# zju3dv/clean-pvnet

Measured on AMD Instinct MI355X. Metric: images/sec RANSAC-vote (480x640, K=9, 512 hyp), higher is better.
Workload: dtype f32; 1 GPU; BASELINE config 3 (cfg3): 480x640, K=9, 512 hypotheses, ~2% foreground, int64 mask, contiguous [B,H,W,K,2] f32 vertex; global batch 64 in contiguous shards of 64 images per GPU; ransac_voting_layer_v3 (+ one RCCL all_gather of [B,K,2] per step for N>1, see extra.exchange); steps cycle over 3 distinct device-resident batches; batch_per_gpu=64, global_batch=64, H=480, W=640, K=9, hn=512, parallelism=batch-sharded x1 (strong scaling: 64 images in total)

## Files before the change

clean-pvnet_amd/csrc/compaction.hpp:

```cpp
#pragma once

struct MaskArgs {
    const void *mask;
    const float *selection;
    int64_t sb, sh, sw;
    int es;
    int contig;
    int mode;
    int W, HW, T;
    int min_num, max_num, cap;
    uint64_t seed;
    int b0;
    int *tn_user;
    int *status;
    int fuse_sub;
    int want_draws;
    const float *seg;
    long long *mask_out;
    int64_t gb, gc, gh, gw;
    int C;
};

constexpr uint32_t kTileNzMask = 0xfffu;

// ... 65 lines not shown

__device__ __forceinline__ float selection_draw(const MaskArgs &a, int b, int p)
{
    if (a.selection) return a.selection[(int64_t)b * a.HW + p];
    return (float)(rng_u32(a.seed, 0u, (uint32_t)(a.b0 + b), (uint32_t)p) >> 8) * 0x1p-24f;
}

__device__ __forceinline__ float list_draw(const MaskArgs &a, int b, int i, int e, const unsigned short *__restrict__ lists ,
                                           const float *__restrict__ draws )
{
    if (draws) return draws[(size_t)i * kTile + e];
    return selection_draw(a, b, i * kTile + (int)lists[(size_t)i * kTile + e]);
}

__device__ __forceinline__ void scan_segments(int *seg)
{
    __syncthreads();
    if (threadIdx.x < 64) {
        const int lane = threadIdx.x;
        const int c = lane < kTileSteps * 4 ? seg[lane] : 0;
        const int inc = wave_incl_scan(c);
        if (lane < kTileSteps * 4) seg[lane] = inc - c;
        if (lane == kTileSteps * 4 - 1) seg[kTileSteps * 4] = inc;
    }
    __syncthreads();
}

template <int ES> struct RawElem;
template <> struct RawElem<1> { typedef uint8_t type; };
template <> struct RawElem<2> { typedef uint16_t type; };
template <> struct RawElem<4> { typedef uint32_t type; };
template <> struct RawElem<8> { typedef uint64_t type; };

template <int ES, bool AHEAD, int MODE , int ST = kElemF32 >
__global__ __launch_bounds__(kBlock) void k_tile_scan(MaskArgs a, uint32_t *__restrict__ tiles,
                                                      unsigned short *__restrict__ tile_list,
                                                      float *__restrict__ tile_draw, int total_tiles)
{
    typedef typename RawElem<ES>::type raw_t;
    __shared__ int seg2[2][kTileSteps * 4 + 1];
    __shared__ int red2[2][4];
    const int lane = lane_id(), wave = threadIdx.x >> 6;
    raw_t cur[AHEAD ? kTileSteps : 1] = {};
    int g = blockIdx.x;
    int b = g / a.T, t = g - b * a.T;
    const int step_b = (int)gridDim.x / a.T, step_t = (int)gridDim.x - step_b * a.T;
    [[maybe_unused]] auto load_tile = [&](raw_t (&dst)[AHEAD ? kTileSteps : 1], int bi, int ti) {
        const raw_t *src = (const raw_t *)a.mask + (int64_t)bi * a.sb + (int64_t)ti * kTile + threadIdx.x;
        if ((ti + 1) * kTile <= a.HW) {
#pragma unroll
            for (int s = 0; s < kTileSteps; ++s) dst[AHEAD ? s : 0] = src[s * kBlock];
        } else {
#pragma unroll
            for (int s = 0; s < kTileSteps; ++s)
                dst[AHEAD ? s : 0] = ti * kTile + s * kBlock + (int)threadIdx.x < a.HW ? src[s * kBlock] : (raw_t)0;
        }
    };
    if constexpr (AHEAD) if (g < total_tiles) load_tile(cur, b, t);
    for (int it = 0; g < total_tiles; ++it) {
        int *seg = seg2[it & 1], *red = red2[it & 1];
        raw_t nxt[AHEAD ? kTileSteps : 1] = {};
        const int gn = g + gridDim.x;
        int bn = b + step_b, tn = t + step_t;
        if (tn >= a.T) { tn -= a.T; ++bn; }
        if constexpr (AHEAD) if (gn < total_tiles) load_tile(nxt, bn, tn);
        unsigned long long m[kTileSteps];
        int pc[kTileSteps];
        int sum = 0;
#pragma unroll
        for (int s = 0; s < kTileSteps; ++s) {
// ... 5 lines not shown
            } else if (p < a.HW) {
                w = mask_weight<ES, ST>(a, b, p);
            }
            m[s] = __ballot(w != 0);
            pc[s] = __popcll(m[s]);
            sum += w;
        }
        if (MODE == 0) sum = wave_total(sum);
        else sum = pc[0] + pc[1] + pc[2] + pc[3] + pc[4] + pc[5] + pc[6] + pc[7];
        if (lane == 0) {
#pragma unroll
            for (int s = 0; s < kTileSteps; ++s) seg[s * 4 + wave] = pc[s];
            red[wave] = sum;
        }
        scan_segments(seg);
        if (threadIdx.x == 0)
            tiles[b * a.T + t] = (uint32_t)seg[kTileSteps * 4] | ((uint32_t)(red[0] + red[1] + red[2] + red[3]) << 12);
        unsigned short *list = tile_list + ((size_t)b * a.T + t) * kTile;
        float *draw = tile_draw + ((size_t)b * a.T + t) * kTile;
        if (seg[kTileSteps * 4] != 0) {
#pragma unroll
            for (int s = 0; s < kTileSteps; ++s)
                if ((m[s] >> lane) & 1ull) {
                    const int r = seg[s * 4 + wave] + __popcll(m[s] & ((1ull << lane) - 1ull));
                    list[r] = (unsigned short)(s * kBlock + threadIdx.x);
                    if (a.want_draws) draw[r] = selection_draw(a, b, t * kTile + s * kBlock + threadIdx.x);
                }
        }
        if constexpr (AHEAD) {
#pragma unroll
            for (int s = 0; s < kTileSteps; ++s) cur[s] = nxt[s];
        }
        g = gn; b = bn; t = tn;
    }
}

typedef float f32x4 __attribute__((ext_vector_type(4)));
typedef long long i64x2 __attribute__((ext_vector_type(2)));
typedef uint32_t u32x2 __attribute__((ext_vector_type(2)));

template <int ST>
__device__ __forceinline__ f32x4 widen_logits4(u32x2 w)
{
    const float2 lo = widen_pair<ST>(w.x), hi = widen_pair<ST>(w.y);
    return f32x4{lo.x, lo.y, hi.x, hi.y};
}

template <bool WRITE_MASK, int ST = kElemF32>
__global__ __launch_bounds__(kBlock) void k_tile_scan_seg2(MaskArgs a, uint32_t *__restrict__ tiles,
                                                           unsigned short *__restrict__ tile_list,
                                                           float *__restrict__ tile_draw)
{
    typedef typename Elem<ST>::raw raw_t;
    __shared__ int seg[8];
    const int g = blockIdx.x;
    const int b = g / a.T, t = g - b * a.T;
    const int lane = lane_id(), wave = threadIdx.x >> 6;
    const raw_t *p0 = (const raw_t *)a.seg + (int64_t)b * a.gb + (int64_t)t * kTile + 4 * threadIdx.x;
    const raw_t *p1 = p0 + a.gc;
    constexpr int kHalf = kTile / 2;
    f32x4 v0[2], v1[2];
    if constexpr (ST == kElemF32) {
#pragma unroll
        for (int s = 0; s < 2; ++s) {
            const bool in = t * kTile + s * kHalf + 4 * (int)threadIdx.x < a.HW;
            v0[s] = in ? __builtin_nontemporal_load((const f32x4 *)(p0 + s * kHalf)) : f32x4{0.f, 0.f, 0.f, 0.f};
// ... 159 lines not shown

__global__ __launch_bounds__(kBlock) void k_tile_subsample(MaskArgs a, uint32_t *__restrict__ tiles,
                                                           unsigned short *__restrict__ tile_list,
                                                           const float *__restrict__ tile_draw)
{
    __shared__ long long redl[4];
    __shared__ int red[8];
    __shared__ int seg[kTileSteps * 4 + 1];
    __shared__ unsigned short keep[kTile];
    const int t = blockIdx.x, b = blockIdx.y;
    const uint32_t w = tiles[b * a.T + t];
    const int nz = (int)(w & kTileNzMask);
    if (nz == 0) return;
    const ImageTotals tot = image_totals(tiles, b, a.T, t, redl, red);
    if (tot.fg <= (long long)a.max_num) return;
    const float prob = (float)a.max_num / (float)tot.fg;
    unsigned short *list = tile_list + ((size_t)b * a.T + t) * kTile;
    const int n = filter_tile_list(a, b, t, nz, prob, tile_list + (size_t)b * a.T * kTile, tile_draw + (size_t)b * a.T * kTile, keep, seg);
    __syncthreads();
    for (int i = threadIdx.x; i < n; i += kBlock) list[i] = keep[i];
    if (threadIdx.x == 0) tiles[b * a.T + t] = (uint32_t)n | (w & ~kTileNzMask);
}

struct VertexArgs {
    const float *vertex;
    int64_t sb, sh, sw, sk, sc;
    int K;
    int vec2;
};

template <int VT> struct VertexRaw { typedef uint2 type; };
template <> struct VertexRaw<kElemF32> { typedef float2 type; };

template <int VT>
__device__ __forceinline__ typename VertexRaw<VT>::type load_vertex(const VertexArgs &v, int b, int y, int x, int vi)
{
    if constexpr (VT == kElemF32) {
        const float *src = v.vertex + (int64_t)b * v.sb + (int64_t)y * v.sh + (int64_t)x * v.sw + (int64_t)vi * v.sk;
        if (v.vec2) return *(const float2 *)src;
        return make_float2(src[0], src[v.sc]);
    } else {
        const uint16_t *src = (const uint16_t *)v.vertex + (int64_t)b * v.sb + (int64_t)y * v.sh + (int64_t)x * v.sw + (int64_t)vi * v.sk;
        if (v.vec2) return make_uint2(*(const uint32_t *)src, 0u);
        return make_uint2(src[0], src[v.sc]);
    }
}

template <int VT>
__device__ __forceinline__ float2 widen_vertex(const VertexArgs &v, typename VertexRaw<VT>::type r)
{
    if constexpr (VT == kElemF32) {
        return r;
    } else {
        typedef typename Elem<VT>::raw raw_t;
        if (v.vec2) return widen_pair<VT>(r.x);
        return make_float2(widen(__builtin_bit_cast(raw_t, (uint16_t)r.x)), widen(__builtin_bit_cast(raw_t, (uint16_t)r.y)));
    }
}

struct HypArgs {
    const int32_t *idxs;
    const int32_t *idxs2;
    int hn, hn_first;
    uint32_t stream, stream2;
    float2 *hyps;
    int *counts;
    int32_t *draws_out;
    int blocks;
    int *surv;
    int *lead;
    int *miss;
};

constexpr int kHypRejectTries = 1 << 12;
constexpr float kSurvMinProb = 1.f / 64.f;
constexpr int kSurvCap = 8192;

__device__ __forceinline__ int select_pixel(const int *prefix, int T, const unsigned short *__restrict__ lists , int t,
                                            size_t *entry = nullptr )
{
    int lo = 0, hi = T - 1;
    while (lo < hi) {
        const int mid = (lo + hi) >> 1;
        if (prefix[mid] > t) hi = mid; else lo = mid + 1;
    }
    const int r = t - (lo ? prefix[lo - 1] : 0);
    const size_t e = (size_t)lo * kTile + r;
    if (entry) *entry = e;
    return lo * kTile + (int)lists[e];
}
// ... 43 lines not shown
        if (fg < (long long)a.min_num) tn = 0;
        const bool sub = a.fuse_sub && fg > (long long)a.max_num;
        const float prob = sub ? (float)a.max_num / (float)fg : 2.f;
        int nsurv = -1;
        if (sub && prob < kSurvMinProb) {
            int *sv = h.surv + (size_t)b * kSurvCap;
            nsurv = 0;
            for (int i = 0; i < a.T; ++i) {
                const int ni = s_prefix[i] - (i ? s_prefix[i - 1] : 0);
                for (int e0 = 0; e0 < ni; e0 += kBlock) {
                    const int e = e0 + threadIdx.x;
                    const bool keep = e < ni && list_draw(a, b, i, e, img_lists, img_draws) < prob;
                    const unsigned long long m = __ballot(keep);
                    __syncthreads();
                    if (lane == 0) red[wave] = __popcll(m);
                    __syncthreads();
                    int off = nsurv;
                    for (int w2 = 0; w2 < wave; ++w2) off += red[w2];
                    off += __popcll(m & ((1ull << lane) - 1ull));
                    if (keep && off < kSurvCap) sv[off] = i * kTile + (int)img_lists[(size_t)i * kTile + e];
                    nsurv += red[0] + red[1] + red[2] + red[3];
                }
            }
            __threadfence_block();
            __syncthreads();
            if (nsurv > kSurvCap) nsurv = -1;
            else if (nsurv < tn) tn = nsurv;
        }

        const int gid = j * kBlock + threadIdx.x;
        if (gid >= v.K * h.hn) return;
        const int vi = gid / h.hn, hi = gid - vi * h.hn;
        const size_t o = ((size_t)b * v.K + vi) * h.hn + hi;
        h.counts[o] = 0;
        if (h.miss) h.miss[o] = 0;
        if (h.lead && hi == 0) {
            int *lw = h.lead + ((size_t)b * v.K + vi) * 8 + 4;
            lw[0] = 0; lw[1] = 0; lw[2] = 0; lw[3] = 0;
        }
        if (tn <= 0) {
            h.hyps[o] = make_float2(0.f, 0.f);
            if (h.draws_out) { h.draws_out[2 * o] = -1; h.draws_out[2 * o + 1] = -1; }
            return;
        }
        const bool first = hi < h.hn_first;
        const int32_t *src = first ? h.idxs : h.idxs2;
        int p0, p1;
        if (src) {
            const int32_t *ip = first ? h.idxs + (((size_t)b * h.hn_first + hi) * v.K + vi) * 2
                                      : h.idxs2 + (((size_t)b * (h.hn - h.hn_first) + (hi - h.hn_first)) * v.K + vi) * 2;
            int t0 = ip[0], t1 = ip[1];
            t0 = t0 < 0 ? 0 : (t0 >= tn ? tn - 1 : t0);
            t1 = t1 < 0 ? 0 : (t1 >= tn ? tn - 1 : t1);
            p0 = select_pixel(s_prefix, a.T, img_lists, t0);
            p1 = select_pixel(s_prefix, a.T, img_lists, t1);
        } else {
            const uint32_t stream = first ? h.stream : h.stream2;
            const uint32_t c = (uint32_t)((first ? hi : hi - h.hn_first) * v.K + vi) * 2u;
            const uint32_t img = (uint32_t)(a.b0 + b);
            if (!sub) {
                p0 = select_pixel(s_prefix, a.T, img_lists, (int)(rng_u32(a.seed, stream, img, c) % (uint32_t)tn));
                p1 = select_pixel(s_prefix, a.T, img_lists, (int)(rng_u32(a.seed, stream, img, c + 1u) % (uint32_t)tn));
            } else if (nsurv >= 0) {
                const int *sv = h.surv + (size_t)b * kSurvCap;
                p0 = sv[rng_u32(a.seed, stream, img, c) % (uint32_t)tn];
                p1 = sv[rng_u32(a.seed, stream, img, c + 1u) % (uint32_t)tn];
            } else {
                p0 = p1 = -1;
                for (int tr = 0; tr < kHypRejectTries && (p0 < 0 || p1 < 0); ++tr) {
                    size_t e;
                    const uint32_t stry = stream + 16u + 4u * (uint32_t)tr;
                    if (p0 < 0) {
                        const int p = select_pixel(s_prefix, a.T, img_lists, (int)(rng_u32(a.seed, stry, img, c) % (uint32_t)total), &e);
                        if ((img_draws ? img_draws[e] : selection_draw(a, b, p)) < prob) p0 = p;
                    }
                    if (p1 < 0) {
                        const int p = select_pixel(s_prefix, a.T, img_lists, (int)(rng_u32(a.seed, stry, img, c + 1u) % (uint32_t)total), &e);
                        if ((img_draws ? img_draws[e] : selection_draw(a, b, p)) < prob) p1 = p;
                    }
                }
                if (p0 < 0 || p1 < 0) {
                    h.hyps[o] = make_float2(0.f, 0.f);
                    if (h.draws_out) { h.draws_out[2 * o] = p0; h.draws_out[2 * o + 1] = p1; }
                    return;
                }
            }
        }
        const int y0 = p0 / a.W, x0 = p0 - y0 * a.W, y1 = p1 / a.W, x1 = p1 - y1 * a.W;
        const typename VertexRaw<VT>::type r0 = load_vertex<VT>(v, b, y0, x0, vi), r1 = load_vertex<VT>(v, b, y1, x1, vi);
        const float2 d0 = widen_vertex<VT>(v, r0), d1 = widen_vertex<VT>(v, r1);
        h.hyps[o] = hypothesis_exact(d0.x, d0.y, (float)x0, (float)y0, d1.x, d1.y, (float)x1, (float)y1);
        if (h.draws_out) { h.draws_out[2 * o] = p0; h.draws_out[2 * o + 1] = p1; }
        return;
    }

    const int t = blockIdx.x - h.blocks;
    const int nz = (int)(tiles[b * a.T + t] & kTileNzMask);
    if (t != 0 && !(a.fuse_sub && t == a.T - 1) && nz == 0) return;
    const unsigned short *my_list = img_lists + (size_t)t * kTile;
    unsigned short mine[kTileSteps];
#pragma unroll
    for (int s = 0; s < kTileSteps; ++s) {
        const int e = s * kBlock + threadIdx.x;
        mine[s] = e < nz ? my_list[e] : (unsigned short)0;
    }
    const ImageTotals tot = image_totals(tiles, b, a.T, t, redl, red);
    if (tot.fg < (long long)a.min_num) {
        if (t == 0 && threadIdx.x == 0) {
            tn_out[b] = 0;
            if (a.tn_user) a.tn_user[b] = 0;
            if (a.status) a.status[b] = PVV_STATUS_SKIPPED;
        }
        return;
    }
    int before = tot.before, tile_n = nz;
    const bool sub = a.fuse_sub && tot.fg > (long long)a.max_num;
    if (sub) {
        const float prob = (float)a.max_num / (float)tot.fg;
        int cnt = 0;
        if (img_draws || a.T > kBlock) {
            for (int i = 0; i < t; ++i) {
                const int ni = (int)(tiles[b * a.T + i] & kTileNzMask);
                for (int e = threadIdx.x; e < ni; e += kBlock)
                    cnt += list_draw(a, b, i, e, img_lists, img_draws) < prob ? 1 : 0;
// ... 40 lines not shown
                }
            }
        }
        before = block_sum(cnt, red);
        __syncthreads();
        tile_n = filter_tile_list(a, b, t, nz, prob, img_lists, img_draws, list, seg);
        __syncthreads();
        if (t == a.T - 1 && threadIdx.x == 0) {
            const int all = before + tile_n;
            tn_out[b] = all < a.cap ? all : a.cap;
            if (a.tn_user) a.tn_user[b] = tn_out[b];
            if (a.status) a.status[b] = PVV_STATUS_SUBSAMPLED | (all > a.cap ? PVV_STATUS_TRUNCATED : 0);
        }
    } else {
        if (t == 0 && threadIdx.x == 0) {
            tn_out[b] = tot.total < a.cap ? tot.total : a.cap;
            if (a.tn_user) a.tn_user[b] = tn_out[b];
            if (a.status) a.status[b] = (tot.fg > (long long)a.max_num ? PVV_STATUS_SUBSAMPLED : 0) |
                                        (tot.total > a.cap ? PVV_STATUS_TRUNCATED : 0);
        }
#pragma unroll
        for (int s = 0; s < kTileSteps; ++s) {
            const int e = s * kBlock + threadIdx.x;
            if (e < nz) list[e] = mine[s];
        }
        __syncthreads();
    }
    const int room = a.cap - before;
    const int n = tile_n < room ? tile_n : (room > 0 ? room : 0);
    constexpr int kKeys = 12;
    for (int li = threadIdx.x; li < n; li += kBlock) {
        const int p = t * kTile + list[li];
        const int y = p / a.W, x = p - y * a.W;
        coords[(size_t)b * a.cap + before + li] = make_float2((float)x, (float)y);
        float2 *drow = dirs + (size_t)b * v.K * a.cap + before + li;
        for (int v0 = 0; v0 < v.K; v0 += kKeys) {
            typename VertexRaw<VT>::type d[kKeys];
#pragma unroll
            for (int u = 0; u < kKeys; ++u)
                if (v0 + u < v.K) d[u] = load_vertex<VT>(v, b, y, x, v0 + u);
#pragma unroll
            for (int u = 0; u < kKeys; ++u)
                if (v0 + u < v.K) {
                    if constexpr (VT == kElemF32) drow[(size_t)(v0 + u) * a.cap] = d[u];
                    else drow[(size_t)(v0 + u) * a.cap] = widen_vertex<VT>(v, d[u]);
                }
        }
    }
}
```

clean-pvnet_amd/csrc/count_prune.hpp:

```cpp
#pragma once

struct LeadArgs {
    const int *tn_arr;
    const float2 *coords;
    const float2 *dirs;
    const float2 *hyps;
    const int *counts;
    int *lead;
    const int *any_staged;
    int K, hn, cap;
    int hstride;
    float kappa, beta, eps;
    int nsplit;
};

constexpr int kLead = 2;

template <uint32_t FIRST>
__global__ __launch_bounds__(kBlock) void k_lead(LeadArgs a)
{
    constexpr uint32_t REST = stage_rest_of(FIRST);
    __shared__ int s_cnt[4], s_idx[4], s_sum[4][4];
    const int vi = blockIdx.x / a.nsplit, split = blockIdx.x - vi * a.nsplit, b = blockIdx.y, bk = b * a.K + vi;
    const int lane = lane_id(), wave = threadIdx.x >> 6;
    constexpr int PC = 4 * kBfPixPerWave;
    if (*a.any_staged == 0) return;
    const int tn = a.tn_arr[b];
    const int nch = (tn + PC - 1) / PC;
    if (tn <= 0 || nch < kStageMinChunks) return;
    constexpr int kTrip = 10;
    const int rem_px = stage_pixels<REST>(tn, nch, PC);
    const int per = (rem_px + a.nsplit - 1) / a.nsplit;
    const int r1 = min(rem_px, (split + 1) * per);
    const float2 *crd = a.coords + (size_t)b * a.cap;
    const float2 *dir = a.dirs + (size_t)bk * a.cap;
    float2 cc[kTrip], dd_[kTrip];
    auto load_trip = [&](int r0) {
#pragma unroll
        for (int u = 0; u < kTrip; ++u) {
            const int r = r0 + u * kBlock;
            cc[u] = dd_[u] = make_float2(0.f, 0.f);
            if (r < r1) {
                const int p = stage_chunk_at<REST>(r / PC) * PC + (r & (PC - 1));
                cc[u] = crd[p];
                dd_[u] = dir[p];
            }
        }
    };
    int r0 = split * per + threadIdx.x;
    load_trip(r0);
    const int *cp = a.counts + (size_t)bk * a.hstride;
    int best = -1, besth = 0x7fffffff;
    for (int h = threadIdx.x; h < a.hn; h += kBlock) {
// ... 63 lines not shown
```

clean-pvnet_amd/csrc/pvnet_vote.hip:

```cpp
#include <hip/hip_runtime.h>

#include <algorithm>
#include <cmath>
#include <cstdio>
#include <cstdlib>
#include <cstring>
#include <mutex>
#include <type_traits>

#include "pvnet_vote.h"

#pragma clang fp contract(off)

#define PVV_EXPORT extern "C" __attribute__((visibility("default")))

namespace {

constexpr int kBlock = 256;
constexpr int kTileSteps = 8;
constexpr int kTile = kBlock * kTileSteps;
constexpr int kFuseSubTiles = 160;
constexpr int kMaxTiles = 16000;
constexpr int kPixPerWave = 64;

// ... 55 lines not shown
Layout make_layout(const pvv_problem *p)
{
    Layout L;
    const size_t HW = (size_t)p->H * p->W;
    L.T = (int)((HW + kTile - 1) / kTile);
    size_t off = 0;
    auto take = [&](size_t bytes) { size_t o = off; off = align_up(off + bytes); return o; };
    L.tiles = take(sizeof(uint32_t) * (size_t)p->B * L.T);
    L.tile_list = take(sizeof(unsigned short) * (size_t)p->B * L.T * kTile);
    L.tile_draw = may_store_draws(p, L.T) ? take(sizeof(float) * (size_t)p->B * L.T * kTile) : 0;
    L.tn = take(sizeof(int) * (size_t)p->B);
    L.surv = take(sizeof(int) * (size_t)p->B * kSurvCap);
    L.coords = take(sizeof(float2) * (size_t)p->B * p->cap);
    L.dirs = take(sizeof(float2) * (size_t)p->B * p->K * p->cap);
    L.hyps = take(sizeof(float2) * (size_t)p->B * p->K * p->hn);
    L.counts = take(sizeof(int) * (size_t)p->B * p->K * p->hn);
    L.sums = take(sizeof(double) * (size_t)p->B * p->K * kRefitSplitMax * 5);
    L.ratio = take(sizeof(float) * (size_t)p->B * p->K);
    L.lead = may_stage(p) ? take(sizeof(int) * 2 * lead_set_words(p)) : 0;
    L.miss = may_stage(p) ? take(sizeof(int) * (size_t)p->B * p->K * p->hn) : 0;
    L.total = off;
    return L;
}

int validate(const pvv_problem *p)
{
    if (!p) return fail(PVV_E_ARG, "problem is NULL");
    if (p->B <= 0 || p->H <= 0 || p->W <= 0 || p->K <= 0 || p->hn <= 0)
        return fail(PVV_E_ARG, "B, H, W, K, hn must be positive");
    if (p->B > kMaxBatchLds) return fail(PVV_E_ARG, "B > 1024: split the batch");
    if (((long long)p->H * p->W + kTile - 1) / kTile > kMaxTiles) return fail(PVV_E_ARG, "H*W too large (more than 16000 tiles of 2048 pixels)");
    if ((long long)p->K * p->hn >= (1ll << 23)) return fail(PVV_E_ARG, "K*hn must be < 2^23");
    if (p->count_kernel < PVV_COUNT_AUTO || p->count_kernel > PVV_COUNT_STAGED_ESTIMATE) return fail(PVV_E_ARG, "unknown count_kernel");
    if (p->flags & ~(PVV_FLAG_DEVICE_RNG | PVV_FLAG_VERTEX_F16 | PVV_FLAG_VERTEX_BF16 | PVV_FLAG_SEG_F16 | PVV_FLAG_SEG_BF16))
        return fail(PVV_E_ARG, "unknown bits in flags");
    if ((p->flags & PVV_FLAG_VERTEX_F16) && (p->flags & PVV_FLAG_VERTEX_BF16))
        return fail(PVV_E_ARG, "flags: PVV_FLAG_VERTEX_F16 and PVV_FLAG_VERTEX_BF16 are exclusive");
    if ((p->flags & PVV_FLAG_SEG_F16) && (p->flags & PVV_FLAG_SEG_BF16))
        return fail(PVV_E_ARG, "flags: PVV_FLAG_SEG_F16 and PVV_FLAG_SEG_BF16 are exclusive");
    if (p->mask_elem_size != 1 && p->mask_elem_size != 2 && p->mask_elem_size != 4 &&
        p->mask_elem_size != 8)
        return fail(PVV_E_ARG, "mask_elem_size must be 1, 2, 4 or 8");
    if (p->cap <= 0 || (long long)p->cap > (long long)p->H * p->W)
        return fail(PVV_E_ARG, "cap must be in [1, H*W]");
    if ((long long)p->B * p->K * p->hn >= (1ll << 31) || (long long)p->B * p->K * p->cap >= (1ll << 40))
        return fail(PVV_E_ARG, "problem too large for one call");
    if (p->singular_policy < PVV_SINGULAR_REFERENCE || p->singular_policy > PVV_SINGULAR_IMAGE_ZERO)
        return fail(PVV_E_ARG, "unknown singular_policy");
    return PVV_OK;
}

int num_cus()
{
    static int cus[64] = {0};
    int dev = 0;
    if (hipGetDevice(&dev) != hipSuccess || dev < 0 || dev >= 64) return 256;
    if (!cus[dev]) {
        hipDeviceProp_t prop;
        int n = 0;
        if (hipGetDeviceProperties(&prop, dev) == hipSuccess) n = prop.multiProcessorCount;
        cus[dev] = n > 0 ? n : 256;
    }
    return cus[dev];
}

int launch_count(const CountArgs &a, hipStream_t st)
{
    const int grid = num_cus() * 8;
// ... 132 lines not shown
    static const double xs[6] = {0.0, 0.585, 1.0, 1.585, 2.0, 3.0}, ys[6] = {0.990, 0.966, 0.957, 0.910, 0.765, 0.50};
    const double x = std::log2(std::max(work, 1.0) / 2.26e10);
    double thr;
    if (x <= xs[0]) thr = ys[0] + (ys[1] - ys[0]) / (xs[1] - xs[0]) * (x - xs[0]);
    else if (x >= xs[5]) thr = ys[5];
    else {
        int i = 0;
        while (x > xs[i + 1]) ++i;
        thr = ys[i] + (ys[i + 1] - ys[i]) * (x - xs[i]) / (xs[i + 1] - xs[i]);
    }
    thr -= 0.1 * std::log2(std::max(p->hn, 512) / 512.0);
    return (float)std::min(0.995, std::max(0.5, thr));
}

double stage_work(const pvv_problem *p, hipStream_t st, float *mean = nullptr, float *max_tn = nullptr)
{
    double sum_tn = -1.0;
    float mt = -1.f;
    const float m = stage_hint_mean(p, st, &mt, &sum_tn);
    if (mean) *mean = m;
    if (max_tn) *max_tn = mt;
    if (m < 0.f || sum_tn < 0.0) return stage_proxy_work(p);
    return (double)p->K * p->hn * sum_tn / kStageProxyFg;
}

bool stage_hint_allows(const pvv_problem *p, hipStream_t st)
{
    if (p->count_kernel != PVV_COUNT_AUTO) return true;
    float max_tn = -1.f, m = -1.f;
    const double work = stage_work(p, st, &m, &max_tn);
    if (work < kStageMinWork) return false;
    if (m < 0.f) return true;
    return m >= stage_hint_threshold(p, work) && max_tn > (float)((kStageMinChunks - 1) * 4 * kBfPixPerWave);
}

Bf16Consts bf16_consts(float thresh)
{
    const double T = (double)thresh, s2 = 1.0 - T * T, kappa = T / std::sqrt(s2);
    const double u = 0x1p-24;
    Bf16Consts fc;
    fc.beta = (float)(1.25 * (33.0 * (1.0 + kappa) + 8.0 / s2) * u / T);
    fc.eps_c = (float)(1.25 * (1.0 + kappa) * 35.0 * u);
    fc.eps0 = (float)(1.5e-6 * (1.0 + kappa));
    fc.kappa = (float)kappa;
    fc.beta2 = (float)(1.25 * (8.0 * (1.0 + kappa) + 8.0 / s2) * u / T);
#ifdef PVV_TUNING
    static const char *dbg = getenv("PVV_DEBUG_BAND_SCALE");
    if (dbg && *dbg) {
        const float k = (float)atof(dbg);
        fc.beta *= k; fc.eps_c *= k; fc.eps0 *= k;
    }
#endif
    return fc;
}

int tuning_int(const char *name, int dflt)
{
#ifdef PVV_TUNING
    static const char *names[32];
    static int vals[32], n = 0;
    for (int i = 0; i < n; ++i) if (!strcmp(names[i], name)) return vals[i] == INT32_MIN ? dflt : vals[i];
    const char *e = getenv(name);
    if (n < 32) { names[n] = name; vals[n] = e && *e ? atoi(e) : INT32_MIN; ++n; }
    return e && *e ? atoi(e) : dflt;
#else
    (void)name;
// ... 38 lines not shown
    const pvv_problem *p = a.p;
    const Layout &L = *a.L;
    char *ws = a.ws;
    hipStream_t st = a.st;
    const Bf16Consts fc = a.fc;
    const float2 *coords = (const float2 *)(ws + L.coords), *dirs = (const float2 *)(ws + L.dirs);
    const float2 *hyps = (const float2 *)(ws + L.hyps) + a.col0;
    int *counts = (int *)(ws + L.counts) + a.col0;
    const int *tn = (const int *)(ws + L.tn);
    int *lead = (int *)(ws + L.lead) + (size_t)a.lead_set * lead_set_words(p);
    StageArgs sa;
    sa.lead = nullptr;
    sa.any_staged = lead + (size_t)p->B * p->K * 8;
    sa.miss = (int *)(ws + L.miss) + a.col0;
    sa.sub_tenth = a.sub_tenth;
    sa.hstride = a.hstride;
    sa.mean = (a.sub_tenth && tuning_int("PVV_PROX", 1) != 0) ? (const float2 *)a.mean : nullptr;
#ifdef PVV_STAMPS
    sa.dbg = tuning_ptr("PVV_DBG_PTR_FILTER");
#endif
    hipLaunchKernelGGL((k_count_bf16<kCountFirst, FIRST>), dim3(a.per_cu_first * num_cus()), dim3(kBlock), 0, st, coords, dirs, hyps, counts, tn,
                       p->B, p->K, p->hn, p->cap, p->inlier_thresh, fc, a.target_first, a.dbg, sa);
    if (int e = check_launch("k_count_bf16<first>")) return e;
    if (int e = mark(p, PVV_MARK_STAGE0, st)) return e;
    LeadArgs la;
    la.tn_arr = tn; la.coords = coords; la.dirs = dirs; la.hyps = hyps; la.counts = counts; la.lead = lead;
    la.K = p->K; la.hn = p->hn; la.cap = p->cap;
    la.hstride = a.hstride > 0 ? a.hstride : p->hn;
    la.kappa = fc.kappa; la.beta = 2.f * fc.beta2; la.eps = 2.f * fc.eps0;
    la.any_staged = sa.any_staged;
    la.nsplit = 16;
    while (la.nsplit > 1 && (long long)p->B * p->K * la.nsplit > 8ll * num_cus()) la.nsplit >>= 1;
    la.nsplit = tuning_int("PVV_LEAD_SPLIT", la.nsplit);
    hipLaunchKernelGGL(k_lead<FIRST>, dim3(p->K * la.nsplit, p->B), dim3(kBlock), 0, st, la);
    if (int e = check_launch("k_lead")) return e;
    if (int e = mark(p, PVV_MARK_PRUNE0, st)) return e;
    sa.lead = lead;
    const long long rest = p->count_kernel == PVV_COUNT_AUTO ? stage_hint_rest_chunks(p, st, stage_rest_of(FIRST)) : -1;
    const bool runs = rest < 0 || rest * p->K >= 2ll * a.target_filter || p->hn > 512;
    if (tuning_int("PVV_FILTER_OLD", runs ? 0 : 1) == 0) {
        hipLaunchKernelGGL(k_count_filter_runs<FIRST>, dim3(tuning_int("PVV_GRID_PER_CU_FILTER", 5) * num_cus()), dim3(kBlock), sizeof(int) * (size_t)p->B, st, coords, dirs,
                           hyps, counts, tn, p->B, p->K, p->hn, p->cap, p->inlier_thresh, fc, a.target_filter, tuning_int("PVV_RUN_R", 0), sa);
        return check_launch("k_count_filter_runs");
    }
    hipLaunchKernelGGL((k_count_bf16<kCountFilter, FIRST>), dim3(a.per_cu_filter * num_cus()), dim3(kBlock), 0, st, coords, dirs, hyps, counts, tn,
                       p->B, p->K, p->hn, p->cap, p->inlier_thresh, fc, a.target_filter, a.dbg, sa);
    return check_launch("k_count_bf16<filter>");
}

struct CountCols {
    int col0 = 0;
    int hstride = 0;
    int lead_set = 0;
    const float *mean = nullptr;
};

int launch_count_bf16(const pvv_problem *p, const Layout &L, char *ws, hipStream_t st, int staged ,
                      const CountCols &cc = CountCols())
{
    const int per_cu_t = tuning_int("PVV_GRID_PER_CU", 0);
    const int items_per_cu = tuning_int("PVV_ITEMS_PER_CU", 5);
    bool few = p->B <= 8;
    if (p->count_kernel == PVV_COUNT_AUTO) {
        double sum_tn = -1.0;
        if (stage_hint_mean(p, st, nullptr, &sum_tn) >= 0.f && sum_tn >= 0.0)
            few = sum_tn / (4 * kBfPixPerWave) * p->K * ((p->hn + 511) / 512) <= 2000.0;
    }
// ... 60 lines not shown
    if (!may_stage(p) || L.lead == 0) return 0;
    if (kind == 1 && stage_hint_allows(p, st)) return 1;
    if (kind == 2 && (p->count_kernel == PVV_COUNT_STAGED_ESTIMATE || (p->count_kernel == PVV_COUNT_AUTO && est_stage_auto(p, st)))) return 2;
    return 0;
}

int launch_count_any(const pvv_problem *p, const Layout &L, char *ws, hipStream_t st, int staged, const CountCols &cc = CountCols())
{
    if (p->ev_count_begin && hipEventRecord((hipEvent_t)p->ev_count_begin, st) != hipSuccess)
        return fail(PVV_E_ARG, "ev_count_begin is not a valid hipEvent_t");
    if (!use_bf16_count(p) && (cc.col0 || cc.hstride)) return fail(PVV_E_ARG, "internal: a column range needs the bf16 count kernel");
    const int e = use_bf16_count(p) ? launch_count_bf16(p, L, ws, st, staged, cc) : launch_count(planar_count_args(p, L, ws), st);
    if (e) return e;
    if (p->ev_count_end && hipEventRecord((hipEvent_t)p->ev_count_end, st) != hipSuccess)
        return fail(PVV_E_ARG, "ev_count_end is not a valid hipEvent_t");
    return PVV_OK;
}

template <int ES, int MODE, int ST = kElemF32>
void launch_scan(const MaskArgs &m, const Layout &L, char *ws, int B, hipStream_t st)
{
    const long long total = (long long)L.T * B;
    uint32_t *tiles = (uint32_t *)(ws + L.tiles);
    unsigned short *lists = (unsigned short *)(ws + L.tile_list);
    float *draws = (float *)(ws + L.tile_draw);
    if (!(m.contig && !m.seg)) {
        hipLaunchKernelGGL((k_tile_scan<ES, false, MODE, ST>), dim3((unsigned)total), dim3(kBlock), 0, st, m, tiles, lists, draws, (int)total);
        return;
    }
    const int per_cu_t = tuning_int("PVV_SCAN_PER_CU", 0);
    long long per_block = 1;
    if (per_cu_t > 0) per_block = (total + (long long)per_cu_t * num_cus() - 1) / ((long long)per_cu_t * num_cus());
    const int grid = (int)((total + per_block - 1) / per_block);
    hipLaunchKernelGGL((k_tile_scan<ES, true, MODE>), dim3(grid), dim3(kBlock), 0, st, m, tiles, lists, draws, (int)total);
}

struct Front {
    MaskArgs m;
    VertexArgs v;
    HypArgs h;
    bool can_subsample;
    bool seg2;
    int vt, st;
    long long *mask_deferred;
};

Front make_front(const pvv_problem *p, int mode, const void *d_mask, const float *d_vertex, const int32_t *d_idxs,
                 const float *d_selection, char *ws, const Layout &L, int32_t *d_tn, const float *d_seg,
                 int64_t *d_mask_out, const int32_t *d_idxs2, int hn_first, uint32_t stream_first, uint32_t stream_rest)
{
    Front f;
    MaskArgs &m = f.m;
    m.mask = d_mask;
    m.seg = d_seg;
    m.mask_out = (long long *)d_mask_out;
    m.gb = p->seg_stride[0]; m.gc = p->seg_stride[1]; m.gh = p->seg_stride[2]; m.gw = p->seg_stride[3];
    m.C = p->seg_classes;
    m.selection = d_selection;
    m.sb = p->mask_stride[0]; m.sh = p->mask_stride[1]; m.sw = p->mask_stride[2];
    m.es = p->mask_elem_size;
    m.contig = (m.sw == 1 && m.sh == p->W) ? 1 : 0;
    m.mode = mode;
    m.W = p->W; m.HW = p->H * p->W; m.T = L.T;
    m.min_num = p->min_num; m.max_num = p->max_num; m.cap = p->cap;
    m.seed = p->seed;
    m.b0 = p->first_image;
    m.tn_user = d_tn;
// ... 584 lines not shown
```

include/pvnet_vote.h:

```cpp
#ifndef PVNET_VOTE_H_
#define PVNET_VOTE_H_

#include <stddef.h>
#include <stdint.h>

#ifdef __cplusplus
extern "C" {
#endif

#define PVV_OK 0
#define PVV_E_ARG (-1)
#define PVV_E_WORKSPACE (-2)

#define PVV_ABI_VERSION 8

int pvv_abi_version(void);
const char *pvv_last_error(void);

int pvv_shutdown(void);


int pvv_generate_hypothesis(const float *d_direct, const float *d_coords,
                            const int32_t *d_idxs, float *d_hypo_pts, int tn,
                            int vn, int hn, void *stream);
// ... 21 lines not shown
                      const float *d_hypo_pts, int32_t *d_counts, int tn,
                      int vn, int hn, float inlier_thresh, void *stream);


typedef struct pvv_problem {
    int32_t B, H, W, K;
    int32_t hn;
    int32_t mask_elem_size;
    int32_t min_num;
    int32_t max_num;
    int32_t cap;
    int32_t singular_policy;
    float inlier_thresh;
    int64_t mask_stride[3];
    int64_t vertex_stride[5];
    uint64_t seed;
    int32_t seg_classes;
    int32_t first_image;
    int64_t seg_stride[4];
    int32_t count_kernel;
    int32_t flags;
    int32_t *d_draws_out;
    void *ev_count_begin;
    void *ev_count_end;
    int32_t *d_status;
    void **ev_marks;
} pvv_problem;

#define PVV_FLAG_DEVICE_RNG 1
#define PVV_FLAG_VERTEX_F16 2
#define PVV_FLAG_VERTEX_BF16 4
#define PVV_FLAG_SEG_F16 8
#define PVV_FLAG_SEG_BF16 16

#define PVV_STATUS_SKIPPED 1
#define PVV_STATUS_SUBSAMPLED 2
#define PVV_STATUS_TRUNCATED 4

#define PVV_MARK_BEGIN 0
#define PVV_MARK_SCAN 1
#define PVV_MARK_COMPACT 2
#define PVV_MARK_COUNT 3
#define PVV_MARK_SELECT 4
#define PVV_MARK_END 5
#define PVV_MARK_STAGE0 6
#define PVV_MARK_PRUNE0 7
#define PVV_N_MARKS 8

#define PVV_COUNT_AUTO 0
#define PVV_COUNT_EXACT 1

#define PVV_COUNT_FULL 2
#define PVV_COUNT_STAGED 3
#define PVV_COUNT_STAGED_ESTIMATE 4

#define PVV_SINGULAR_REFERENCE 0
#define PVV_SINGULAR_ZERO 1
#define PVV_SINGULAR_IMAGE_ZERO 2

int32_t pvv_default_cap(int32_t H, int32_t W, int32_t max_num);

size_t pvv_workspace_bytes(const pvv_problem *p);

int pvv_ransac_voting_v3(const pvv_problem *p, const void *d_mask,
                         const float *d_vertex, const int32_t *d_idxs,
                         const float *d_selection, void *d_workspace,
// ... 44 lines not shown
```

Before: 331,800 images/s.

## Add wide 16-byte mask scan, nontemporal compaction stores, adaptive lead count

```diff
diff --git a/clean-pvnet_amd/csrc/compaction.hpp b/clean-pvnet_amd/csrc/compaction.hpp
--- a/clean-pvnet_amd/csrc/compaction.hpp
+++ b/clean-pvnet_amd/csrc/compaction.hpp
@@ -121,10 +121,107 @@
 template <> struct RawElem<4> { typedef uint32_t type; };
 template <> struct RawElem<8> { typedef uint64_t type; };
 
-template <int ES, bool AHEAD, int MODE , int ST = kElemF32 >
-__global__ __launch_bounds__(kBlock) void k_tile_scan(MaskArgs a, uint32_t *__restrict__ tiles,
-                                                      unsigned short *__restrict__ tile_list,
-                                                      float *__restrict__ tile_draw, int total_tiles)
+typedef unsigned long long u64x2 __attribute__((ext_vector_type(2)));
+constexpr int kWideSteps = kTileSteps / 2;
+
+__device__ __forceinline__ unsigned wave_incl_scan(unsigned v)
+{
+    v += (unsigned)PVV_DPP(0, (int)v, 0x111, 0xf, true);
+    v += (unsigned)PVV_DPP(0, (int)v, 0x112, 0xf, true);
+    v += (unsigned)PVV_DPP(0, (int)v, 0x114, 0xf, true);
+    v += (unsigned)PVV_DPP(0, (int)v, 0x118, 0xf, true);
+    v += (unsigned)PVV_DPP(0, (int)v, 0x142, 0xa, false);
+    v += (unsigned)PVV_DPP(0, (int)v, 0x143, 0xc, false);
+    return v;
+}
+
+template <int MODE>
+__device__ __forceinline__ void tile_scan_wide(const MaskArgs &a, uint32_t *__restrict__ tiles, unsigned short *__restrict__ tile_list,
+                                               float *__restrict__ tile_draw, int total_tiles)
+{
+    static_assert(kWideSteps * 8 <= 32 && 2 * 64 < 256, "four byte-wide counts in one word");
+    __shared__ int seg2[2][kTileSteps * 4 + 1];
+    __shared__ int red2[2][4];
+    const int lane = lane_id(), wave = threadIdx.x >> 6;
+    u64x2 cur[kWideSteps] = {};
+    int g = blockIdx.x;
+    int b = g / a.T, t = g - b * a.T;
+    const int step_b = (int)gridDim.x / a.T, step_t = (int)gridDim.x - step_b * a.T;
+    auto load_tile = [&](u64x2 (&dst)[kWideSteps], int bi, int ti) {
+        const uint64_t *base = (const uint64_t *)a.mask + (int64_t)bi * a.sb + (int64_t)ti * kTile;
+        const uint64_t *src = base + 2 * threadIdx.x;
+        if ((ti + 1) * kTile <= a.HW && ((uintptr_t)base & 15) == 0) {
+#pragma unroll
+            for (int s = 0; s < kWideSteps; ++s) dst[s] = *(const u64x2 *)(src + s * 2 * kBlock);
+        } else {
+#pragma unroll
+            for (int s = 0; s < kWideSteps; ++s) {
+                const int p = ti * kTile + s * 2 * kBlock + 2 * (int)threadIdx.x;
+                dst[s].x = p < a.HW ? src[s * 2 * kBlock] : 0ull;
+                dst[s].y = p + 1 < a.HW ? src[s * 2 * kBlock + 1] : 0ull;
+            }
+        }
+    };
+    if (g < total_tiles) load_tile(cur, b, t);
+    for (int it = 0; g < total_tiles; ++it) {
+        int *seg = seg2[it & 1], *red = red2[it & 1];
+        u64x2 nxt[kWideSteps] = {};
+        const int gn = g + gridDim.x;
+        int bn = b + step_b, tn = t + step_t;
+        if (tn >= a.T) { tn -= a.T; ++bn; }
+        if (gn < total_tiles) load_tile(nxt, bn, tn);
+        unsigned fg = 0u;
+        unsigned packed = 0u;
+        int sum = 0;
+#pragma unroll
+        for (int s = 0; s < kWideSteps; ++s)
+#pragma unroll
+            for (int j = 0; j < 2; ++j) {
+                const uint64_t v = cur[s][j];
+                const int w = MODE == 0 ? (int)(v & 0xFF) : (v == 1 ? 1 : 0);
+                const unsigned f = w != 0 ? 1u : 0u;
+                fg |= f << (2 * s + j);
+                packed += f << (8 * s);
+                sum += w;
+            }
+        const unsigned inc = wave_incl_scan(packed);
+        const unsigned excl = inc - packed;
+        const unsigned tot = (unsigned)__builtin_amdgcn_readlane((int)inc, 63);
+        if (MODE == 0) sum = wave_total(sum);
+        else sum = (int)((tot & 0xff) + ((tot >> 8) & 0xff) + ((tot >> 16) & 0xff) + (tot >> 24));
+        if (lane == 0) {
+#pragma unroll
+            for (int s = 0; s < kTileSteps; ++s) seg[s * 4 + wave] = s < kWideSteps ? (int)((tot >> (8 * s)) & 0xff) : 0;
+            red[wave] = sum;
+        }
+        scan_segments(seg);
+        if (threadIdx.x == 0)
+            tiles[b * a.T + t] = (uint32_t)seg[kTileSteps * 4] | ((uint32_t)(red[0] + red[1] + red[2] + red[3]) << 12);
+        unsigned short *list = tile_list + ((size_t)b * a.T + t) * kTile;
+        float *draw = tile_draw + ((size_t)b * a.T + t) * kTile;
+        if (seg[kTileSteps * 4] != 0 && fg != 0u) {
+#pragma unroll
+            for (int s = 0; s < kWideSteps; ++s) {
+                int r = seg[s * 4 + wave] + (int)((excl >> (8 * s)) & 0xff);
+#pragma unroll
+                for (int j = 0; j < 2; ++j)
+                    if ((fg >> (2 * s + j)) & 1u) {
+                        const int off = s * 2 * kBlock + 2 * (int)threadIdx.x + j;
+                        list[r] = (unsigned short)off;
+                        if (a.want_draws) draw[r] = selection_draw(a, b, t * kTile + off);
+                        ++r;
+                    }
+            }
+        }
+#pragma unroll
+        for (int s = 0; s < kWideSteps; ++s) cur[s] = nxt[s];
+        g = gn; b = bn; t = tn;
+    }
+}
+
+template <int ES, bool AHEAD, int MODE , int ST >
+__device__ __forceinline__ void tile_scan_narrow(const MaskArgs &a, uint32_t *__restrict__ tiles, unsigned short *__restrict__ tile_list,
+                                                 float *__restrict__ tile_draw, int total_tiles)
 {
     typedef typename RawElem<ES>::type raw_t;
     __shared__ int seg2[2][kTileSteps * 4 + 1];
@@ -196,6 +293,20 @@
             for (int s = 0; s < kTileSteps; ++s) cur[s] = nxt[s];
         }
         g = gn; b = bn; t = tn;
+    }
+}
+
+template <int ES, bool AHEAD, int MODE, int ST = kElemF32,
+          bool WIDE = false >
+__global__ __launch_bounds__(kBlock) void k_tile_scan(MaskArgs a, uint32_t *__restrict__ tiles,
+                                                      unsigned short *__restrict__ tile_list,
+                                                      float *__restrict__ tile_draw, int total_tiles)
+{
+    if constexpr (WIDE) {
+        static_assert(ES == 8 && AHEAD, "the wide scan is the read-ahead scan of 8-byte elements");
+        tile_scan_wide<MODE>(a, tiles, tile_list, tile_draw, total_tiles);
+    } else {
+        tile_scan_narrow<ES, AHEAD, MODE, ST>(a, tiles, tile_list, tile_draw, total_tiles);
     }
 }
 
@@ -421,11 +532,20 @@
 template <int VT> struct VertexRaw { typedef uint2 type; };
 template <> struct VertexRaw<kElemF32> { typedef float2 type; };
 
-template <int VT>
+#ifdef PVV_COMPACT_NT_GATHER
+constexpr bool kGatherStream = true;
+#else
+constexpr bool kGatherStream = false;
+#endif
+template <int VT, bool STREAM = false>
 __device__ __forceinline__ typename VertexRaw<VT>::type load_vertex(const VertexArgs &v, int b, int y, int x, int vi)
 {
     if constexpr (VT == kElemF32) {
         const float *src = v.vertex + (int64_t)b * v.sb + (int64_t)y * v.sh + (int64_t)x * v.sw + (int64_t)vi * v.sk;
+        if constexpr (STREAM) {
+            typedef float gx2 __attribute__((ext_vector_type(2)));
+            if (v.vec2) { const gx2 r = __builtin_nontemporal_load((const gx2 *)src); return make_float2(r.x, r.y); }
+        }
         if (v.vec2) return *(const float2 *)src;
         return make_float2(src[0], src[v.sc]);
     } else {
@@ -445,6 +565,26 @@
         if (v.vec2) return widen_pair<VT>(r.x);
         return make_float2(widen(__builtin_bit_cast(raw_t, (uint16_t)r.x)), widen(__builtin_bit_cast(raw_t, (uint16_t)r.y)));
     }
+}
+
+typedef float f32x2 __attribute__((ext_vector_type(2)));
+__device__ __forceinline__ void store_row(float2 *dst, float2 v)
+{
+#ifdef PVV_COMPACT_PLAIN_STORE
+    *dst = v;
+#else
+    __builtin_nontemporal_store(f32x2{v.x, v.y}, (f32x2 *)dst);
+#endif
+}
+
+template <typename T>
+__device__ __forceinline__ void store_word(T *dst, T v)
+{
+#ifdef PVV_COMPACT_SMALL_NT
+    __builtin_nontemporal_store(v, dst);
+#else
+    *dst = v;
+#endif
 }
 
 struct HypArgs {
@@ -554,8 +694,8 @@
         if (gid >= v.K * h.hn) return;
         const int vi = gid / h.hn, hi = gid - vi * h.hn;
         const size_t o = ((size_t)b * v.K + vi) * h.hn + hi;
-        h.counts[o] = 0;
-        if (h.miss) h.miss[o] = 0;
+        store_word(&h.counts[o], 0);
+        if (h.miss) store_word(&h.miss[o], 0);
         if (h.lead && hi == 0) {
             int *lw = h.lead + ((size_t)b * v.K + vi) * 8 + 4;
             lw[0] = 0; lw[1] = 0; lw[2] = 0; lw[3] = 0;
@@ -611,7 +751,12 @@
         const int y0 = p0 / a.W, x0 = p0 - y0 * a.W, y1 = p1 / a.W, x1 = p1 - y1 * a.W;
         const typename VertexRaw<VT>::type r0 = load_vertex<VT>(v, b, y0, x0, vi), r1 = load_vertex<VT>(v, b, y1, x1, vi);
         const float2 d0 = widen_vertex<VT>(v, r0), d1 = widen_vertex<VT>(v, r1);
-        h.hyps[o] = hypothesis_exact(d0.x, d0.y, (float)x0, (float)y0, d1.x, d1.y, (float)x1, (float)y1);
+        const float2 hyp = hypothesis_exact(d0.x, d0.y, (float)x0, (float)y0, d1.x, d1.y, (float)x1, (float)y1);
+#ifdef PVV_COMPACT_SMALL_NT
+        __builtin_nontemporal_store(f32x2{hyp.x, hyp.y}, (f32x2 *)&h.hyps[o]);
+#else
+        h.hyps[o] = hyp;
+#endif
         if (h.draws_out) { h.draws_out[2 * o] = p0; h.draws_out[2 * o + 1] = p1; }
         return;
     }
@@ -718,18 +863,18 @@
     for (int li = threadIdx.x; li < n; li += kBlock) {
         const int p = t * kTile + list[li];
         const int y = p / a.W, x = p - y * a.W;
-        coords[(size_t)b * a.cap + before + li] = make_float2((float)x, (float)y);
+        store_row(coords + (size_t)b * a.cap + before + li, make_float2((float)x, (float)y));
         float2 *drow = dirs + (size_t)b * v.K * a.cap + before + li;
         for (int v0 = 0; v0 < v.K; v0 += kKeys) {
             typename VertexRaw<VT>::type d[kKeys];
 #pragma unroll
             for (int u = 0; u < kKeys; ++u)
-                if (v0 + u < v.K) d[u] = load_vertex<VT>(v, b, y, x, v0 + u);
+                if (v0 + u < v.K) d[u] = load_vertex<VT, kGatherStream>(v, b, y, x, v0 + u);
 #pragma unroll
             for (int u = 0; u < kKeys; ++u)
                 if (v0 + u < v.K) {
-                    if constexpr (VT == kElemF32) drow[(size_t)(v0 + u) * a.cap] = d[u];
-                    else drow[(size_t)(v0 + u) * a.cap] = widen_vertex<VT>(v, d[u]);
+                    if constexpr (VT == kElemF32) store_row(drow + (size_t)(v0 + u) * a.cap, d[u]);
+                    else store_row(drow + (size_t)(v0 + u) * a.cap, widen_vertex<VT>(v, d[u]));
                 }
         }
     }
diff --git a/clean-pvnet_amd/csrc/count_prune.hpp b/clean-pvnet_amd/csrc/count_prune.hpp
--- a/clean-pvnet_amd/csrc/count_prune.hpp
+++ b/clean-pvnet_amd/csrc/count_prune.hpp
@@ -14,11 +14,10 @@
     int nsplit;
 };
 
-constexpr int kLead = 2;
-
-template <uint32_t FIRST>
+template <uint32_t FIRST, int kLead>
 __global__ __launch_bounds__(kBlock) void k_lead(LeadArgs a)
 {
+    static_assert(kLead == 1 || kLead == 2, "one or two leaders");
     constexpr uint32_t REST = stage_rest_of(FIRST);
     __shared__ int s_cnt[4], s_idx[4], s_sum[4][4];
     const int vi = blockIdx.x / a.nsplit, split = blockIdx.x - vi * a.nsplit, b = blockIdx.y, bk = b * a.K + vi;
diff --git a/clean-pvnet_amd/csrc/pvnet_vote.hip b/clean-pvnet_amd/csrc/pvnet_vote.hip
--- a/clean-pvnet_amd/csrc/pvnet_vote.hip
+++ b/clean-pvnet_amd/csrc/pvnet_vote.hip
@@ -111,8 +111,11 @@
     if (((long long)p->H * p->W + kTile - 1) / kTile > kMaxTiles) return fail(PVV_E_ARG, "H*W too large (more than 16000 tiles of 2048 pixels)");
     if ((long long)p->K * p->hn >= (1ll << 23)) return fail(PVV_E_ARG, "K*hn must be < 2^23");
     if (p->count_kernel < PVV_COUNT_AUTO || p->count_kernel > PVV_COUNT_STAGED_ESTIMATE) return fail(PVV_E_ARG, "unknown count_kernel");
-    if (p->flags & ~(PVV_FLAG_DEVICE_RNG | PVV_FLAG_VERTEX_F16 | PVV_FLAG_VERTEX_BF16 | PVV_FLAG_SEG_F16 | PVV_FLAG_SEG_BF16))
+    if (p->flags & ~(PVV_FLAG_DEVICE_RNG | PVV_FLAG_VERTEX_F16 | PVV_FLAG_VERTEX_BF16 | PVV_FLAG_SEG_F16 | PVV_FLAG_SEG_BF16 |
+                     PVV_FLAG_LEAD_ONE | PVV_FLAG_LEAD_TWO))
         return fail(PVV_E_ARG, "unknown bits in flags");
+    if ((p->flags & PVV_FLAG_LEAD_ONE) && (p->flags & PVV_FLAG_LEAD_TWO))
+        return fail(PVV_E_ARG, "flags: PVV_FLAG_LEAD_ONE and PVV_FLAG_LEAD_TWO are exclusive");
     if ((p->flags & PVV_FLAG_VERTEX_F16) && (p->flags & PVV_FLAG_VERTEX_BF16))
         return fail(PVV_E_ARG, "flags: PVV_FLAG_VERTEX_F16 and PVV_FLAG_VERTEX_BF16 are exclusive");
     if ((p->flags & PVV_FLAG_SEG_F16) && (p->flags & PVV_FLAG_SEG_BF16))
@@ -311,6 +314,18 @@
     if (work < kStageMinWork) return false;
     if (m < 0.f) return true;
     return m >= stage_hint_threshold(p, work) && max_tn > (float)((kStageMinChunks - 1) * 4 * kBfPixPerWave);
+}
+
+constexpr float kLeadOneMinRatio = 0.99f;
+int lead_count(const pvv_problem *p, hipStream_t st)
+{
+    if (p->flags & PVV_FLAG_LEAD_ONE) return 1;
+    if (p->flags & PVV_FLAG_LEAD_TWO) return 2;
+#ifdef PVV_LEAD_ALWAYS_TWO
+    return 2;
+#endif
+    if (p->count_kernel != PVV_COUNT_AUTO) return 2;
+    return stage_hint_mean(p, st) >= kLeadOneMinRatio ? 1 : 2;
 }
 
 Bf16Consts bf16_consts(float thresh)
@@ -415,7 +430,8 @@
     la.nsplit = 16;
     while (la.nsplit > 1 && (long long)p->B * p->K * la.nsplit > 8ll * num_cus()) la.nsplit >>= 1;
     la.nsplit = tuning_int("PVV_LEAD_SPLIT", la.nsplit);
-    hipLaunchKernelGGL(k_lead<FIRST>, dim3(p->K * la.nsplit, p->B), dim3(kBlock), 0, st, la);
+    if (lead_count(p, st) == 1) hipLaunchKernelGGL((k_lead<FIRST, 1>), dim3(p->K * la.nsplit, p->B), dim3(kBlock), 0, st, la);
+    else hipLaunchKernelGGL((k_lead<FIRST, 2>), dim3(p->K * la.nsplit, p->B), dim3(kBlock), 0, st, la);
     if (int e = check_launch("k_lead")) return e;
     if (int e = mark(p, PVV_MARK_PRUNE0, st)) return e;
     sa.lead = lead;
@@ -542,7 +558,12 @@
     long long per_block = 1;
     if (per_cu_t > 0) per_block = (total + (long long)per_cu_t * num_cus() - 1) / ((long long)per_cu_t * num_cus());
     const int grid = (int)((total + per_block - 1) / per_block);
-    hipLaunchKernelGGL((k_tile_scan<ES, true, MODE>), dim3(grid), dim3(kBlock), 0, st, m, tiles, lists, draws, (int)total);
+#ifndef PVV_SCAN_NARROW
+    constexpr bool wide = ES == 8;
+#else
+    constexpr bool wide = false;
+#endif
+    hipLaunchKernelGGL((k_tile_scan<ES, true, MODE, kElemF32, wide>), dim3(grid), dim3(kBlock), 0, st, m, tiles, lists, draws, (int)total);
 }
 
 struct Front {
diff --git a/include/pvnet_vote.h b/include/pvnet_vote.h
--- a/include/pvnet_vote.h
+++ b/include/pvnet_vote.h
@@ -77,6 +77,8 @@
 #define PVV_FLAG_VERTEX_BF16 4
 #define PVV_FLAG_SEG_F16 8
 #define PVV_FLAG_SEG_BF16 16
+#define PVV_FLAG_LEAD_ONE 64
+#define PVV_FLAG_LEAD_TWO 128
 
 #define PVV_STATUS_SKIPPED 1
 #define PVV_STATUS_SUBSAMPLED 2
```

Measured after the change: 329,700 images/s. No clear change (-0.7%).
